# zju-vipa/ProtoPFormer

Measured on AMD Instinct MI355X. Metric: images/sec train step, deit_small+2000 protos, bs256, 1/2/4/8 MI355X, higher is better.
Workload: dtype bf16; 1 GPU; deit_small_patch16_224, synthetic 224x224, 2000x384 prototypes, 200 classes, k=81, batch 256/GPU (BASELINE.json configs[2]), train step = fwd+CE+PPC+bwd+allreduce+AdamW+EMA, DropPath 0.1; blocks after the token reservation run compacted on the 1+k reserved rows (equal to the masked full-length blocks to bf16 rounding); bf16 backbone: the reserved tokens differ from the fp32 reference's in ~2-3 % o; global_batch=256, parallelism=dp1

## Files before the change

include/ppf_hip.h:

```cpp
#ifndef PPF_HIP_H
#define PPF_HIP_H

#include <stddef.h>
#include <stdint.h>

#ifdef __cplusplus
extern "C" {
#endif

typedef struct ihipStream_t* ppf_stream_t;

#define PPF_ERR_SHAPE (-1)
#define PPF_ERR_ALIGN (-2)
#define PPF_ERR_ARG (-3)

#define PPF_ABI_VERSION 10

const char* ppf_last_error(void);
int ppf_abi_version(void);
int ppf_device_info(int* cu_count, int* clock_mhz, char* name, int name_len);
int ppf_stream_arm(ppf_stream_t stream, int on);
int ppf_stream_wait_stream(ppf_stream_t dst, ppf_stream_t src);
int64_t ppf_stream_mark(ppf_stream_t stream);
int ppf_stream_wait_mark(ppf_stream_t stream, int64_t ticket);

int ppf_gemm_bf16(const void* A, const void* B, void* C, int M, int N, int K, int lda, int ldb, int ldc, int trans_a,
                  int trans_b, int epi, const float* bias, const float* res, int ldres, const float* rowscale,
                  int rows_per_group, const float* colscale, const void* aux_in, void* aux_out, int ldaux, float* colsum,
                  float alpha, void* workspace, size_t workspace_bytes, ppf_stream_t stream);
size_t ppf_gemm_workspace_bytes(int M, int N, int K);

int ppf_gemm_test_force_g224(int force);

int ppf_gemm_probe(int enable);
int ppf_gemm_probe_read(double* ms_total, int64_t* launches, double* flops, double* bytes);

int ppf_path_probe(int enable);
int ppf_path_probe_read(int tag, double* ms_total, int64_t* launches, double* flops, double* bytes);

int ppf_gemm_bf16_batched(const void* A, const void* B, void* C, int M, int N, int K, int lda, int ldb, int ldc, int trans_a,
                          int trans_b, int out_f32, float alpha, int batch_outer, int batch_inner, int64_t sa_o, int64_t sa_i,
                          int64_t sb_o, int64_t sb_i, int64_t sc_o, int64_t sc_i, int kpad, ppf_stream_t stream);

int ppf_layernorm_bwd_f32(const float* dy, const float* x, const int* row_map, const float* w, const float* dres_in, float* dx_out, float* dw, float* db,
                          int rows, int D, float eps, ppf_stream_t stream);
int ppf_ew_bwd_f32(int kind, const float* a, const float* b, float* out, const float* rowscale, int rows_per_group, int M, int N, ppf_stream_t stream);
int ppf_colsum_f32(const float* in, float* out, int M, int N, ppf_stream_t stream);
int ppf_attn_bwd_f32(const float* qkv, const float* dout, const float* policy, float* dqkv, float* scratch, int B, int H, int N, int D, int self_keep,
                     int eps_n, ppf_stream_t stream);
int ppf_th_attn_bwd_f32(const float* qkv, const float* dout, const float* wl, const float* bl, const float* ww, const float* bw, float* dqkv,
                        float* dwl, float* dbl, float* dww, float* dbw, int B, int H, int N, int D, ppf_stream_t stream);
int ppf_class_attn_bwd_f32(const float* q, const float* k, const float* v, const float* policy, const float* dout, float* dq, float* dk, float* dv,
                           int B, int H, int N1, int D, ppf_stream_t stream);
// ... 163 lines not shown
```

protopformer_amd/_lib.py:

```python
import ctypes
import os

import torch

_HERE = os.path.dirname(os.path.abspath(__file__))
LIB_PATH = os.environ.get("PPF_LIB_PATH") or os.path.join(_HERE, "lib", "libppf_hip.so")

SIGS = {
    "ppf_gemm_bf16": "pppiiiiiiiiippipipppipf" "pz" "s",
    "ppf_device_info": "pppi",
    "ppf_rowgemm_bf16": "pp" "iiiiii" "pp" "s",
    "ppf_rowgemm_resid_ln": "pp" "iiiiii" "p" "pp" "pi" "pp" "pp" "ppp" "f" "s",
    "ppf_rowgemm_lnbwd": "pp" "iiiiii" "pppp" "ppp" "pi" "pp" "pz" "s",
    "ppf_rowgemm_colsum": "p" "iii" "ppp" "s",
    "ppf_layernorm_bwd_f32": "pppppppp" "ii" "f" "s",
    "ppf_ew_bwd_f32": "i" "ppp" "p" "i" "ii" "s",
    "ppf_colsum_f32": "pp" "ii" "s",
    "ppf_attn_bwd_f32": "ppppp" "iiiiii" "s",
    "ppf_th_attn_bwd_f32": "ppppppp" "pppp" "iiii" "s",
    "ppf_class_attn_bwd_f32": "pppppppp" "iiii" "s",
    "ppf_transpose_bf16_batched": "ppp" "ii" "s",
    "ppf_gemm_probe": "i",
    "ppf_gemm_test_force_g224": "i",
    "ppf_gemm_probe_read": "pppp",
    "ppf_path_probe": "i",
    "ppf_path_probe_read": "ipppp",
    "ppf_layernorm_fwd": "ppppppp" "iif" "s",
    "ppf_layernorm_bwd": "pppppp" "pppp" "pp" "i" "pppp" "ii" "pz" "s",
    "ppf_layernorm_bwd_reduce": "p" "ii" "pppp" "s",
    "ppf_cast_f32_bf16": "ppls",
    "ppf_cast_bf16_f32": "ppls",
    "ppf_im2col_patch": "ppiiiiis",
# ... 64 lines not shown

_CT = {"p": ctypes.c_void_p, "i": ctypes.c_int, "l": ctypes.c_int64, "L": ctypes.c_uint64, "f": ctypes.c_float, "s": ctypes.c_void_p, "z": ctypes.c_size_t}
_lib = None
_FAST = {}
_stream_override = []


def lib():
    global _lib
    if _lib is None:
        if not os.path.exists(LIB_PATH):
            raise RuntimeError(f"{LIB_PATH} not found: build it with `python -m protopformer_amd.build` "
                               "(there is no fallback path)")
        _lib = ctypes.CDLL(LIB_PATH)
        _lib.ppf_last_error.restype = ctypes.c_char_p
        _lib.ppf_abi_version.restype = ctypes.c_int
        got = _lib.ppf_abi_version()
        if got != EXPECTED_ABI:
            _lib = None
            raise RuntimeError(f"{LIB_PATH} was built for ABI version {got}, this binding expects {EXPECTED_ABI}: rebuild it with "
                               "`python -m protopformer_amd.build --force` (a stale library would receive shifted arguments)")
        _lib.ppf_gemm_workspace_bytes.restype = ctypes.c_size_t
        _lib.ppf_gemm_workspace_bytes.argtypes = [ctypes.c_int] * 3
        _lib.ppf_sgemm_pair_workspace.restype = ctypes.c_int64
        _lib.ppf_sgemm_pair_workspace.argtypes = [ctypes.c_int] * 5
        _lib.ppf_proto_bwd_single_workspace.restype = ctypes.c_size_t
        _lib.ppf_proto_bwd_single_workspace.argtypes = [ctypes.c_int] * 3
        _lib.ppf_proto_bwd_workspace.restype = ctypes.c_size_t
        _lib.ppf_proto_fwd_workspace.restype = ctypes.c_size_t
        _lib.ppf_proto_fwd_workspace.argtypes = [ctypes.c_int] * 2
        _lib.ppf_proto_bwd_workspace.argtypes = [ctypes.c_int] * 6
        _lib.ppf_layernorm_bwd_blocks.restype = ctypes.c_int
        _lib.ppf_layernorm_bwd_blocks.argtypes = [ctypes.c_int]
        _lib.ppf_sigmoid_bwd_blocks.restype = ctypes.c_int
        _lib.ppf_sigmoid_bwd_blocks.argtypes = [ctypes.c_int]
        _lib.ppf_clip_grad_blocks.restype = ctypes.c_int
        _lib.ppf_clip_grad_blocks.argtypes = []
        _lib.ppf_rowgemm_supported.restype = ctypes.c_int
        _lib.ppf_rowgemm_supported.argtypes = [ctypes.c_int] * 3
        _lib.ppf_attn_fwd_hm_supported.restype = ctypes.c_int
        _lib.ppf_attn_fwd_hm_supported.argtypes = [ctypes.c_int] * 3
        _lib.ppf_th_fused_supported.restype = ctypes.c_int
        _lib.ppf_th_fused_supported.argtypes = [ctypes.c_int] * 3
        _lib.ppf_th_grads_supported.restype = ctypes.c_int
        _lib.ppf_th_grads_supported.argtypes = [ctypes.c_int] * 3
        _lib.ppf_th_bwd_partial_floats.restype = ctypes.c_size_t
# ... 163 lines not shown
```

protopformer_amd/backbone.py:

```python
import functools
import os

import torch
import torch.nn as nn

from . import _lib, ops
from .ops import EPI_ATOMIC, EPI_BF16, EPI_DGELU, EPI_F32, EPI_GELU, EPI_RESID, EPI_SIGMOID_F32

LN_EPS = 1e-6
_KEEP_CACHE = {}
_ROW_BWD_MAX_ELEMS = 12_000_000


def _row_bwd(M, D):
    return M * D <= _ROW_BWD_MAX_ELEMS


def droppath_scales(rates, B, device, training):
    slots = [r if training else 0.0 for r in rates]
    active = [i for i, r in enumerate(slots) if r > 0.0]
    if not active:
        return None, [-1] * len(slots)
    key = (tuple(slots), str(device))
    st = _KEEP_CACHE.get(key)
# ... 153 lines not shown
        h = ops.linear_f32(h, c.weight, c.bias, kind=2 if j == len(convs) - 2 else 4)
    return h, acts


def addon_bwd(ppnet, store, head, f, df):
    convs = addon_convs(ppnet)
    gv = store.grad_view
    if len(convs) == 1:
        return ops.sigmoid_bwd(df, f, gv(convs[0].bias))
    acts = head["chain"]
    d = ops.ew_bwd_f32(1, df.contiguous(), f)
    for j in reversed(range(1, len(convs))):
        c, x_in = convs[j], acts[j - 1]
        ops.linear_wgrad_f32(d, x_in, gv(c.weight), gv(c.bias))
        d = ops.ew_bwd_f32(5, ops.linear_dgrad_f32(d, c.weight), x_in)
    ops.colsum_f32(d, gv(convs[0].bias))
    return ops.cast_bf16(d)


class WgradLane:

    def __init__(self, device):
        self.enabled = os.environ.get("PPF_WGRAD_STREAM", "1") != "0"
        self.streams = [torch.cuda.Stream(device=device)] if self.enabled else []
        self.raws = [st.cuda_stream for st in self.streams]
        self.last_read = {}
        self.tracked = set()
        self.held = []
        self.pending = []

    def track(self, t):
        self.tracked.add(t.data_ptr())
        return t

    def submit(self, fn, reads, tag=None, defer=False):
        if not self.enabled:
            fn()
            return
        self.pending.append((fn, reads, tag))
        self.held.extend(reads)
        if not defer:
            self.flush()

    def flush(self, tag=None):
        if not self.pending:
            return
        raw = self.raws[0]
        try:
            _lib.call("ppf_stream_wait_stream", raw, _lib.stream_ptr())
            for fn, reads, tg in self.pending:
                _lib.push_stream(raw)
                try:
                    fn()
                    ptrs = [t.data_ptr() for t in reads if t.data_ptr() in self.tracked]
                    if ptrs:
                        ticket = _lib.stream_mark(raw)
                        for q in ptrs:
                            self.last_read[q] = ticket
                finally:
                    _lib.pop_stream()
        finally:
            self.pending.clear()

    def before_overwrite(self, t):
        if t.data_ptr() not in self.tracked:
            raise RuntimeError("WgradLane.before_overwrite: buffer was not registered with track()")
        q = t.data_ptr()
        if any(r.data_ptr() == q for _, reads, _t in self.pending for r in reads):
            self.flush()
        ticket = self.last_read.pop(q, None)
        if ticket is not None:
            _lib.call("ppf_stream_wait_mark", _lib.stream_ptr(), ticket)

    def join(self):
        if self.enabled:
            self.flush()
            for raw in self.raws:
                _lib.call("ppf_stream_wait_stream", _lib.stream_ptr(), raw)
        self.last_read.clear()
        self.tracked.clear()
        self.held.clear()


def wgrad_lane(store):
    lane = getattr(store, "_wgrad_lane", None)
    if lane is None:
        lane = store._wgrad_lane = WgradLane(store.device)
    return lane


_ROLL_TAIL = 1
_ROLL_BATCH = 3


def _wgrad(store, dy16, x16, weight, bias=None, defer=False):
    gw = store.grad_view(weight)
    gb = store.grad_view(bias) if bias is not None else None
    wgrad_lane(store).submit(lambda: ops.gemm(dy16, x16, trans_a=True, trans_b=True, epi=EPI_ATOMIC, out=gw.reshape(weight.shape[0], -1),
                                              colsum=gb), (dy16, x16), defer=defer and min(weight.shape[0], weight.shape[1]) <= 256)


_DGRAD_ROW = 3


def _dgrad(store, dy16, weight, rows, which):
    wt = store.w16t(weight)
    if wt is not None and (_DGRAD_ROW & which) and ops.rowgemm_ok(wt.shape[0], wt.shape[1], rows):
        return ops.rowgemm_bf16(dy16, wt, rows)
    if wt is not None:
        return ops.gemm(dy16, wt, epi=EPI_BF16)
    return ops.gemm(dy16, store.w16(weight), trans_b=True, epi=EPI_BF16)


def head_bwd(ppnet, store, saved, df):
    head = saved["head"]
    conv = addon_convs(ppnet)[0]
    dz = addon_bwd(ppnet, store, head, saved["f"].reshape(-1, saved["f"].shape[-1]), df)
    _wgrad(store, dz, head["nf"], conv.weight)
    return ops.gemm(dz, store.w16(conv.weight).reshape(conv.out_channels, -1), trans_b=True, epi=EPI_BF16)


def chunk_ready(gs, lane, chunk):
# ... 187 lines not shown
```

protopformer_amd/csrc/gemm_bf16.hip:

```cpp
#include "ppf_common.h"
#include "gemm_common.h"
#include <cstdlib>
#include <utility>
#include <vector>

namespace {
using namespace ppfg;

constexpr int BM = 128, BN = 128, BK = 64, NTHREADS = 256;
constexpr int TILE_BYTES = BM * BK * 2;
constexpr int STAGE_LD = 68;
constexpr int STAGE_BYTES = 4 * 32 * STAGE_LD * 4;


__device__ __forceinline__ int lds_off_mode0(int r, int c16) { return r * 128 + ((c16 ^ ((r >> 1) & 7)) << 4); }
template <int ROWS>
__device__ __forceinline__ int lds_off_mode1(int kc, int col) {
    return kc * (ROWS * 2) + ((((col >> 5) ^ (kc & 3))) << 6) + ((col & 31) << 1);
}

typedef uint32_t u32x4 __attribute__((ext_vector_type(4)));

template <bool T, int ROWS>
struct TileIO {
// ... 94 lines not shown
            }
        }
    } else {
        const int col = (lane & 15) * 4;
        const int n = nbase + col;
        const EpiCols cc = epi_load_cols<EPI>(p, n, n < p.N);
        EpiRow rr[8];
#pragma unroll
        for (int pass = 0; pass < 8; ++pass) {
            const int m = mbase + pass * 4 + (lane >> 4);
            rr[pass] = epi_load_row<EPI>(p, m, n, m < p.M && n < p.N);
        }
#pragma unroll
        for (int pass = 0; pass < 8; ++pass) {
            const int r = pass * 4 + (lane >> 4);
            const int m = mbase + r;
            const float4 v = *reinterpret_cast<const float4*>(stage + r * STAGE_LD + col);
            if (m < p.M && n < p.N) epi_store<EPI>(p, m, n, v.x, v.y, v.z, v.w, cc, rr[pass]);
        }
    }
}

template <bool TA, bool TB, int EPI, bool COLSUM, int MT>
__global__ __launch_bounds__(NTHREADS, MT == 2 ? 3 : 2) void gemm_kernel(const GemmParams p_) {
    constexpr int PD = 1;
    extern __shared__ __attribute__((aligned(16))) unsigned char smem[];
    constexpr int TBM = 64 * MT;
    constexpr int A_BYTES = TBM * BK * 2;
    using IOA = TileIO<TA, TBM>;
    using IOB = TileIO<TB, BN>;
    const int tid = threadIdx.x, lane = tid & 63, wave = tid >> 6;
    const int wm = (wave & 1) * (32 * MT), wn = (wave >> 1) * 64;

    const int tiles_n = (p_.N + BN - 1) / BN;
    const int tiles = tiles_n * ((p_.M + TBM - 1) / TBM);
    const int vid_all = xcd_remap(blockIdx.x, gridDim.x);
    const int zslice = vid_all / tiles, vid = vid_all - zslice * tiles;
    const int m0 = (vid / tiles_n) * TBM, n0 = (vid % tiles_n) * BN;
    GemmParams p = p_;
    p.zslice = zslice;
    if (gridDim.y > 1) {
        const int bo = blockIdx.y / p.batch_inner, bi = blockIdx.y % p.batch_inner;
        p.A += bo * p.sa_o + bi * p.sa_i;
        p.B += bo * p.sb_o + bi * p.sb_i;
        const long long co = bo * p.sc_o + bi * p.sc_i;
        p.C = (EPI == EPI_BF16) ? (void*)(reinterpret_cast<bf16_t*>(p.C) + co) : (void*)(reinterpret_cast<float*>(p.C) + co);
    }

    const int nsplit = p.nsplit;
    const int kchunk = (((p.K + nsplit - 1) / nsplit) + BK - 1) / BK * BK;
    const int kbeg = zslice * kchunk;
    const int kend = min(p.K, kbeg + kchunk);
    if (kbeg >= kend) return;
    const int nk = (kend - kbeg + BK - 1) / BK;

    u32x4 ra[PD][IOA::NLD], rb[PD][IOB::NLD];
    unsigned ma[PD], mb[PD];
    f32x16 acc[2][MT];
#pragma unroll
// ... 70 lines not shown
#pragma unroll
    for (int mi = 0; mi < MT; ++mi) {
#pragma unroll
        for (int ni = 0; ni < 2; ++ni)
#pragma unroll
            for (int g = 0; g < 4; ++g)
                *reinterpret_cast<float4*>(stage + (lane & 31) * STAGE_LD + 32 * ni + 8 * g + 4 * h) =
                    make_float4(acc[ni][mi][4 * g], acc[ni][mi][4 * g + 1], acc[ni][mi][4 * g + 2], acc[ni][mi][4 * g + 3]);
        __builtin_amdgcn_wave_barrier();
        epilogue_rows<EPI>(p, stage, m0 + wm + 32 * mi, n0 + wn, lane);
        __builtin_amdgcn_wave_barrier();
        if constexpr (COLSUM) {
            const int m = m0 + wm + 32 * mi + (lane & 31);
            if (do_colsum && h == 0 && m < p.M) {
                if constexpr (EPI == EPI_PARTIAL) {
                    float* dst = p.ws + p.zslice * ((size_t)p.M * p.N + (size_t)p.cs_parts * p.M) + (size_t)p.M * p.N + m;
                    *dst = accs[mi][0];
                } else unsafeAtomicAdd(p.colsum + m, accs[mi][0]);
            }
        }
    }
}

template <int ROWS, int NTHR>
struct TileT {
    static constexpr int CPR = ROWS / 8;
    static constexpr int KPP = NTHR / CPR;
    static constexpr int NLD = BK / KPP;
    static __device__ __forceinline__ unsigned gload(u32x4 (&reg)[NLD], const bf16_t* __restrict__ X, int ld, int R, int row0, int k0, int kend, int tid) {
        const int c16 = tid % CPR, kb = tid / CPR;
        const int col = row0 + c16 * 8;
        const bool cok = (col + 8) <= R;
        const int cc = cok ? col : 0;
        unsigned mask = 0;
#pragma unroll
        for (int i = 0; i < NLD; ++i) {
            const int kc = k0 + kb + KPP * i;
            reg[i] = *reinterpret_cast<const u32x4*>(X + (size_t)min(kc, kend - 1) * ld + cc);
            mask |= (cok && kc < kend) ? (1u << i) : 0u;
        }
        return mask;
    }
    static __device__ __forceinline__ void sstore(const u32x4 (&reg)[NLD], unsigned mask, unsigned char* tile, int tid) {
        const u32x4 zero = {0u, 0u, 0u, 0u};
        const int c16 = tid % CPR, kb = tid / CPR;
#pragma unroll
        for (int i = 0; i < NLD; ++i)
            *reinterpret_cast<u32x4*>(tile + lds_off_mode1<ROWS>(kb + KPP * i, c16 * 8)) = ((mask >> i) & 1u) ? reg[i] : zero;
    }
    static __device__ __forceinline__ bf16x8 frag(const unsigned char* tile, int rbase, int ks, int lane) { return TileIO<true, ROWS>::frag(tile, rbase, ks, lane); }
};

template <int WMW, int WNW, bool COLSUM>
__global__ __launch_bounds__(64 * WMW * WNW, 1) void wgrad8_kernel(const GemmParams p_) {
    extern __shared__ __attribute__((aligned(16))) unsigned char smem[];
    constexpr int NTHR = 64 * WMW * WNW, TBM = 64 * WMW, TBN = 64 * WNW;
    using IOA = TileT<TBM, NTHR>;
    using IOB = TileT<TBN, NTHR>;
    const int tid = threadIdx.x, lane = tid & 63;
    const int wave = __builtin_amdgcn_readfirstlane(tid >> 6);
    const int wm = (wave % WMW) * 64, wn = (wave / WMW) * 64;
    const int tiles_n = (p_.N + TBN - 1) / TBN;
    const int tiles = tiles_n * ((p_.M + TBM - 1) / TBM);
    const int vid_all = xcd_remap(blockIdx.x, gridDim.x);
    const int zslice = vid_all / tiles, vid = vid_all - zslice * tiles;
    const int m0 = (vid / tiles_n) * TBM, n0 = (vid % tiles_n) * TBN;
    GemmParams p = p_;
    p.zslice = zslice;
    const int nsplit = p.nsplit;
    const int kchunk = (((p.K + nsplit - 1) / nsplit) + BK - 1) / BK * BK;
    const int kbeg = zslice * kchunk;
    const int kend = min(p.K, kbeg + kchunk);
    if (kbeg >= kend) return;
    const int nk = (kend - kbeg + BK - 1) / BK;

    u32x4 ra[IOA::NLD], rb[IOB::NLD];
    unsigned ma, mb;
    f32x16 acc[2][2];
#pragma unroll
    for (int i = 0; i < 2; ++i)
#pragma unroll
        for (int j = 0; j < 2; ++j)
#pragma unroll
            for (int r = 0; r < 16; ++r) acc[i][j][r] = 0.f;
    f32x16 accs[2];
    if constexpr (COLSUM) {
#pragma unroll
// ... 44 lines not shown
        __syncthreads();
    }
    const int h = lane >> 5;
    float* stage = reinterpret_cast<float*>(smem) + wave * (32 * STAGE_LD);
#pragma unroll
    for (int mi = 0; mi < 2; ++mi) {
#pragma unroll
        for (int ni = 0; ni < 2; ++ni)
#pragma unroll
            for (int g = 0; g < 4; ++g)
                *reinterpret_cast<float4*>(stage + (lane & 31) * STAGE_LD + 32 * ni + 8 * g + 4 * h) =
                    make_float4(acc[ni][mi][4 * g], acc[ni][mi][4 * g + 1], acc[ni][mi][4 * g + 2], acc[ni][mi][4 * g + 3]);
        __builtin_amdgcn_wave_barrier();
        epilogue_rows<EPI_PARTIAL>(p, stage, m0 + wm + 32 * mi, n0 + wn, lane);
        __builtin_amdgcn_wave_barrier();
        if constexpr (COLSUM) {
            const int m = m0 + wm + 32 * mi + (lane & 31);
            if (do_colsum && h == 0 && m < p.M) {
                float* dst = p.ws + p.zslice * ((size_t)p.M * p.N + (size_t)p.cs_parts * p.M) + (size_t)p.M * p.N + m;
                *dst = accs[mi][0];
            }
        }
    }
}

template <int WMW, int WNW>
int launch_wgrad8(const GemmParams& p, int splitk, hipStream_t stream) {
    auto kern = wgrad8_kernel<WMW, WNW, true>;
    constexpr int NTHR = 64 * WMW * WNW, TBM = 64 * WMW, TBN = 64 * WNW;
    constexpr int opnd = (TBM + TBN) * BK * 2, strips = (NTHR / 64) * 32 * STAGE_LD * 4;
    constexpr int lds = opnd > strips ? opnd : strips;
    static bool attr_set = false;
    if (!attr_set) {
        hipError_t e = hipFuncSetAttribute(reinterpret_cast<const void*>(kern), hipFuncAttributeMaxDynamicSharedMemorySize, lds);
        if (e != hipSuccess) { ppf_set_error("hipFuncSetAttribute(wgrad8): %s", hipGetErrorString(e)); return (int)e; }
        attr_set = true;
    }
    const int tiles = ((p.M + TBM - 1) / TBM) * ((p.N + TBN - 1) / TBN);
    hipLaunchKernelGGL(kern, dim3(tiles * splitk), dim3(NTHR), lds, stream, p);
    PPF_LAUNCH_CHECK();
    return 0;
}

typedef __attribute__((address_space(3))) void g4_lds_t;
typedef const __attribute__((address_space(1))) void g4_gbl_t;

// ... 212 lines not shown
    constexpr int TBM = 64 * MT;
    const int tiles = ((p.M + TBM - 1) / TBM) * ((p.N + BN - 1) / BN);
    auto kern = gemm_kernel<TA, TB, EPI, COLSUM, MT>;
    constexpr int opnd = TBM * BK * 2 + TILE_BYTES;
    constexpr int lds = opnd > STAGE_BYTES ? opnd : STAGE_BYTES;
    static bool attr_set = false;
    if (!attr_set) {
        hipError_t e = hipFuncSetAttribute(reinterpret_cast<const void*>(kern), hipFuncAttributeMaxDynamicSharedMemorySize, lds);
        if (e != hipSuccess) { ppf_set_error("hipFuncSetAttribute(gemm): %s", hipGetErrorString(e)); return (int)e; }
        attr_set = true;
    }
    GemmParams q = p;
    q.nsplit = splitk;
    hipLaunchKernelGGL(kern, dim3(tiles * splitk, nbatch, 1), dim3(NTHREADS), lds, stream, q);
    PPF_LAUNCH_CHECK();
    return 0;
}

template <bool TA, bool TB, int EPI, bool COLSUM>
int launch(const GemmParams& p, int splitk, hipStream_t stream, int nbatch = 1) {
    return launch_impl<TA, TB, EPI, COLSUM, 2>(p, splitk, stream, nbatch);
}

__global__ __launch_bounds__(256) void splitk_reduce_kernel(const float* __restrict__ ws, float* __restrict__ C, float* __restrict__ colsum,
                                                            int M, int N, int ldc, int nsplit, int cs_parts) {
    const size_t mn = (size_t)M * N, slice = mn + (colsum ? (size_t)cs_parts * M : 0);
    const size_t total4 = mn / 4;
    const size_t i = (size_t)blockIdx.x * 256 + threadIdx.x;
    if (i < total4) {
        const float* p = ws + i * 4;
        float4 acc = make_float4(0.f, 0.f, 0.f, 0.f);
        for (int z0 = 0; z0 < nsplit; z0 += 16) {
            float4 v[16];
#pragma unroll
            for (int u = 0; u < 16; ++u) {
                const int z = min(z0 + u, nsplit - 1);
                v[u] = *reinterpret_cast<const float4*>(p + (size_t)z * slice);
            }
#pragma unroll
            for (int u = 0; u < 16; ++u)
                if (z0 + u < nsplit) { acc.x += v[u].x; acc.y += v[u].y; acc.z += v[u].z; acc.w += v[u].w; }
        }
        const size_t e = i * 4, m = e / N, n = e - m * N;
        float4* dst = reinterpret_cast<float4*>(C + m * ldc + n);
        const float4 c = *dst;
        *dst = make_float4(c.x + acc.x, c.y + acc.y, c.z + acc.z, c.w + acc.w);
    } else if (colsum && i < total4 + (size_t)M) {
        const size_t m = i - total4;
        float a = 0.f;
        for (int z = 0; z < nsplit; ++z)
            for (int q = 0; q < cs_parts; ++q) a += ws[(size_t)z * slice + mn + (size_t)q * M + m];
        colsum[m] += a;
    }
}

struct Probe {
    bool on = false;
    std::vector<std::pair<hipEvent_t, hipEvent_t>> pool;
    size_t used = 0;
    double flops = 0.0, bytes = 0.0;
    std::pair<hipEvent_t, hipEvent_t> acquire() {
        if (used == pool.size()) {
            hipEvent_t a = nullptr, b = nullptr;
            const unsigned fl = hipEventDisableSystemFence;
            (void)hipEventCreateWithFlags(&a, fl); (void)hipEventCreateWithFlags(&b, fl);
            pool.emplace_back(a, b);
        }
        return pool[used++];
    }
};
Probe g_probe;

constexpr size_t PPF_GEMM_COUNTER_BYTES = 16384;

int pick_splitk(int M, int N, int K) {
    const int tiles = ((M + BM - 1) / BM) * ((N + BN - 1) / BN);
    const int target = min(M, N) <= 256 ? 216 : 432;
    int s = target / tiles;
    const int maxs = (K + 4 * BK - 1) / (4 * BK);
    if (s > maxs) s = maxs;
    if (s < 1) s = 1;
    const int kchunk = (((K + s - 1) / s) + BK - 1) / BK * BK;
    return (K + kchunk - 1) / kchunk;
}

}

extern "C" {

int ppf_gemm_test_force_g224(int force) { g_force_g224 = force != 0; return 0; }

size_t ppf_gemm_workspace_bytes(int M, int N, int K) {
    return PPF_GEMM_COUNTER_BYTES + (size_t)pick_splitk(M, N, K) * ((size_t)M * N + M) * sizeof(float);
}

int ppf_gemm_bf16(const void* A, const void* B, void* C, int M, int N, int K, int lda, int ldb, int ldc, int trans_a,
                  int trans_b, int epi, const float* bias, const float* res, int ldres, const float* rowscale,
                  int rows_per_group, const float* colscale, const void* aux_in, void* aux_out, int ldaux, float* colsum,
                  float alpha, void* workspace, size_t workspace_bytes, hipStream_t stream) {
    PPF_CHECK_ARG(M > 0 && N > 0 && K > 0, PPF_ERR_SHAPE, "ppf_gemm_bf16: bad shape M=%d N=%d K=%d", M, N, K);
    PPF_CHECK_ARG((lda % 8) == 0 && (ldb % 8) == 0 && (ldc % 4) == 0 && (N % 4) == 0, PPF_ERR_ALIGN,
                  "ppf_gemm_bf16: lda/ldb must be multiples of 8, ldc and N of 4 (lda=%d ldb=%d ldc=%d N=%d)", lda, ldb, ldc, N);
    PPF_CHECK_ARG(trans_a ? (M % 8 == 0) : (K % 8 == 0), PPF_ERR_ALIGN, "ppf_gemm_bf16: A inner extent must be a multiple of 8");
    PPF_CHECK_ARG(trans_b ? (N % 8 == 0) : (K % 8 == 0), PPF_ERR_ALIGN, "ppf_gemm_bf16: B inner extent must be a multiple of 8");
    PPF_CHECK_ARG((((uintptr_t)A | (uintptr_t)B | (uintptr_t)C) & 15) == 0, PPF_ERR_ALIGN, "ppf_gemm_bf16: pointers must be 16-byte aligned");
    PPF_CHECK_ARG(!(trans_a && !trans_b), PPF_ERR_ARG, "ppf_gemm_bf16: (trans_a=1, trans_b=0) is not instantiated");
    PPF_CHECK_ARG((((uintptr_t)aux_in | (uintptr_t)aux_out | (uintptr_t)res) & 15) == 0 && (ldaux % 4) == 0 && (ldres % 4) == 0, PPF_ERR_ALIGN,
// ... 24 lines not shown
            case EPI_SIGMOID_F32: return launch<false, false, EPI_SIGMOID_F32, false>(p, 1, stream);
            case EPI_RESID: return launch<false, false, EPI_RESID, false>(p, 1, stream);
            case EPI_DGELU: return launch<false, false, EPI_DGELU, false>(p, 1, stream);
            default: break;
        }
    } else if (!trans_a && trans_b) {
        switch (epi) {
            case EPI_BF16: return launch<false, true, EPI_BF16, false>(p, 1, stream);
            case EPI_F32: return launch<false, true, EPI_F32, false>(p, 1, stream);
            case EPI_DGELU: return launch<false, true, EPI_DGELU, false>(p, 1, stream);
            default: break;
        }
    } else {
        switch (epi) {
            case EPI_ATOMIC: {
                const int ns = pick_splitk(M, N, K);
                const size_t need = PPF_GEMM_COUNTER_BYTES + (size_t)ns * ((size_t)M * N + M) * sizeof(float);
                if (workspace == nullptr || workspace_bytes < need || ns == 1) return launch<true, true, EPI_ATOMIC, true>(p, ns, stream);
                p.ws = (float*)((unsigned char*)workspace + PPF_GEMM_COUNTER_BYTES);
                p.cs_parts = 1;
                p.nsplit = ns;
                hipEvent_t e0 = nullptr, e1 = nullptr;
                if (g_probe.on) { auto ev = g_probe.acquire(); e0 = ev.first; e1 = ev.second; (void)hipEventRecord(e0, stream); }
                const bool wide = (M < N ? M : N) >= 320;
                int rc;
                if (wide && M >= 512 && M >= N && (M % 256 == 0 || M >= 1024)) rc = launch_wgrad8<4, 2>(p, ns, stream);
                else if (wide && N >= 512 && (N % 256 == 0 || N >= 1024)) rc = launch_wgrad8<2, 4>(p, ns, stream);
                else rc = launch<true, true, EPI_PARTIAL, true>(p, ns, stream);
                if (rc) return rc;
                if (g_probe.on) {
                    (void)hipEventRecord(e1, stream);
                    g_probe.flops += 2.0 * M * N * (double)K;
                    g_probe.bytes += 2.0 * ((double)M * K + (double)N * K) + 4.0 * M * N;
                }
                const size_t work = (size_t)M * N / 4 + (colsum ? M : 0);
                const int grid = (int)((work + 255) / 256);
                hipLaunchKernelGGL(splitk_reduce_kernel, dim3(grid), dim3(256), 0, stream, p.ws, (float*)C, colsum, M, N, ldc, ns, p.cs_parts);
                PPF_LAUNCH_CHECK();
                return 0;
            }
            case EPI_F32: return launch<true, true, EPI_F32, false>(p, 1, stream);
            default: break;
        }
    }
    ppf_set_error("ppf_gemm_bf16: combination trans_a=%d trans_b=%d epi=%d not instantiated", trans_a, trans_b, epi);
    return PPF_ERR_ARG;
}

int ppf_gemm_probe(int enable) {
    if (enable == 1) { g_probe.used = 0; g_probe.flops = 0.0; g_probe.bytes = 0.0; }
    if (enable == 2) {
        for (auto& e : g_probe.pool) { (void)hipEventDestroy(e.first); (void)hipEventDestroy(e.second); }
        g_probe.pool.clear(); g_probe.used = 0;
    }
    g_probe.on = enable == 1;
    return 0;
}
int ppf_gemm_probe_read(double* ms_total, int64_t* launches, double* flops, double* bytes) {
    double ms = 0.0;
    for (size_t i = 0; i < g_probe.used; ++i) {
        auto& e = g_probe.pool[i];
        float t = 0.f;
        hipError_t rc = hipEventSynchronize(e.second);
        if (rc == hipSuccess) rc = hipEventElapsedTime(&t, e.first, e.second);
        if (rc != hipSuccess) { ppf_set_error("ppf_gemm_probe_read: %s", hipGetErrorString(rc)); return (int)rc; }
        ms += t;
    }
    if (ms_total) *ms_total = ms;
    if (launches) *launches = (int64_t)g_probe.used;
// ... 39 lines not shown
```

protopformer_amd/ops.py:

```python
import os

import torch

from . import _lib

EPI_BF16, EPI_F32, EPI_GELU, EPI_SIGMOID_F32, EPI_RESID, EPI_DGELU, EPI_ATOMIC = range(7)


DOMINANT_NAME = ("weight-gradient bf16 MFMA GEMM, split over the contraction, ordered partial tiles: wgrad8_kernel<4,2> / <2,4> (256x128 / 128x256 tiles) "
                 "and gemm_kernel<TA=1,TB=1,EPI_PARTIAL,COLSUM> (128x128)")


_WORKSPACE = {}


def _workspace(device, nbytes):
    key = (device, _lib.stream_ptr())
    buf = _WORKSPACE.get(key)
    if buf is None or buf.numel() < nbytes:
        if buf is not None:
            _RETIRED_WS.append(buf)
        buf = torch.empty(max(nbytes, 64 << 20), dtype=torch.uint8, device=device)
        _WORKSPACE[key] = buf
    return buf


_GEMM_WS = {}
_RETIRED_WS = []


def _gemm_workspace(device, nbytes):
    key = (device, _lib.stream_ptr())
    buf = _GEMM_WS.get(key)
# ... 17 lines not shown
    _chk(a, torch.bfloat16), _chk(b, torch.bfloat16)
    lda = a.shape[1] if lda is None else lda
    ldb = b.shape[1] if ldb is None else ldb
    M, K = (a.shape[1], a.numel() // lda) if trans_a else (a.numel() // lda, a.shape[1])
    N, Kb = (b.shape[1], b.numel() // ldb) if trans_b else (b.numel() // ldb, b.shape[1])
    assert K == Kb, f"contraction mismatch {K} vs {Kb}"
    if out is None:
        odt = torch.float32 if epi in (EPI_F32, EPI_SIGMOID_F32, EPI_RESID, EPI_ATOMIC) else torch.bfloat16
        out = torch.empty((M, N), dtype=odt, device=a.device)
        if epi == EPI_ATOMIC:
            zero_(out)
    ldaux = 0
    for t in (aux_in, aux_out):
        if t is not None:
            _chk(t, torch.uint8 if epi in (EPI_GELU, EPI_DGELU) else torch.bfloat16)
            ldaux = t.shape[-1]
    ws = None
    if epi == EPI_ATOMIC and workspace:
        ws = _gemm_workspace(a.device, _lib.lib().ppf_gemm_workspace_bytes(M, N, K))
    _lib.call("ppf_gemm_bf16", a, b, out, M, N, K, lda, ldb, out.shape[-1], int(trans_a), int(trans_b), epi,
              bias, res, res.shape[-1] if res is not None else 0, rowscale, rows_per_group, colscale, aux_in, aux_out, ldaux,
              colsum, float(alpha), ws, ws.numel() if ws is not None else 0)
    return out


def rowgemm_ok(D, K, rows_per_tile):
    return bool(_lib.lib().ppf_rowgemm_supported(int(D), int(K), int(rows_per_tile)))


_CU_COUNT = {}


def rowgemm_tile_rows(M, rows_per_sample, device=None, backward=False):
    dev = torch.cuda.current_device() if device is None else device
    cus = _CU_COUNT.get(dev)
    if cus is None:
        cus = _CU_COUNT[dev] = torch.cuda.get_device_properties(dev).multi_processor_count
    tiles = (M + rows_per_sample - 1) // rows_per_sample
    if 3 * tiles > 2 * cus or rows_per_sample <= 16:
        return rows_per_sample
    half = (rows_per_sample + 1) // 2
    if backward:
        target = max(1, int(0.62 * cus))
        return max(half, min(rows_per_sample, (M + target - 1) // target))
    return half

# ... 666 lines not shown
```

Before: 17530 images/sec.

## Fuse pairs of weight-gradient GEMMs into one grouped split-K launch

Adds a paired weight-gradient kernel that runs two split-K GEMMs in a single grid, splitting the blocks between them, followed by one combined split-K reduction kernel. The split factors are chosen jointly, in proportion to each problem's FLOPs, against a CU-sized slot target. The wgrad lane now defers submissions and merges adjacent jobs into pairs. This cuts launch count and lets small GEMMs share the device instead of each underfilling it. In exchange, jobs are held back longer on the side stream, which may reduce overlap, and the new split factors and larger workspace may be less tuned than the single-GEMM heuristics.

```diff
diff --git a/include/ppf_hip.h b/include/ppf_hip.h
--- a/include/ppf_hip.h
+++ b/include/ppf_hip.h
@@ -29,6 +29,12 @@
                   int rows_per_group, const float* colscale, const void* aux_in, void* aux_out, int ldaux, float* colsum,
                   float alpha, void* workspace, size_t workspace_bytes, ppf_stream_t stream);
 size_t ppf_gemm_workspace_bytes(int M, int N, int K);
+
+int ppf_gemm_bf16_wgrad_pair(const void* A0, const void* B0, void* C0, int M0, int N0, int K0, int lda0, int ldb0, int ldc0, float* colsum0,
+                             const void* A1, const void* B1, void* C1, int M1, int N1, int K1, int lda1, int ldb1, int ldc1, float* colsum1,
+                             void* workspace, size_t workspace_bytes, ppf_stream_t stream);
+size_t ppf_gemm_workspace_pair_bytes(int M0, int N0, int K0, int M1, int N1, int K1);
+int ppf_gemm_test_pair_target(int target);
 
 int ppf_gemm_test_force_g224(int force);
 
diff --git a/protopformer_amd/_lib.py b/protopformer_amd/_lib.py
--- a/protopformer_amd/_lib.py
+++ b/protopformer_amd/_lib.py
@@ -8,6 +8,8 @@
 
 SIGS = {
     "ppf_gemm_bf16": "pppiiiiiiiiippipipppipf" "pz" "s",
+    "ppf_gemm_bf16_wgrad_pair": "ppp" "iiiiii" "p" "ppp" "iiiiii" "p" "pz" "s",
+    "ppf_gemm_test_pair_target": "i",
     "ppf_device_info": "pppi",
     "ppf_rowgemm_bf16": "pp" "iiiiii" "pp" "s",
     "ppf_rowgemm_resid_ln": "pp" "iiiiii" "p" "pp" "pi" "pp" "pp" "ppp" "f" "s",
@@ -118,6 +120,8 @@
                                "`python -m protopformer_amd.build --force` (a stale library would receive shifted arguments)")
         _lib.ppf_gemm_workspace_bytes.restype = ctypes.c_size_t
         _lib.ppf_gemm_workspace_bytes.argtypes = [ctypes.c_int] * 3
+        _lib.ppf_gemm_workspace_pair_bytes.restype = ctypes.c_size_t
+        _lib.ppf_gemm_workspace_pair_bytes.argtypes = [ctypes.c_int] * 6
         _lib.ppf_sgemm_pair_workspace.restype = ctypes.c_int64
         _lib.ppf_sgemm_pair_workspace.argtypes = [ctypes.c_int] * 5
         _lib.ppf_proto_bwd_single_workspace.restype = ctypes.c_size_t
diff --git a/protopformer_amd/backbone.py b/protopformer_amd/backbone.py
--- a/protopformer_amd/backbone.py
+++ b/protopformer_amd/backbone.py
@@ -199,6 +199,7 @@
 
     def __init__(self, device):
         self.enabled = os.environ.get("PPF_WGRAD_STREAM", "1") != "0"
+        self.pair = self.enabled and os.environ.get("PPF_WGRAD_PAIR", "1") != "0"
         self.streams = [torch.cuda.Stream(device=device)] if self.enabled else []
         self.raws = [st.cuda_stream for st in self.streams]
         self.last_read = {}
@@ -210,11 +211,20 @@
         self.tracked.add(t.data_ptr())
         return t
 
-    def submit(self, fn, reads, tag=None, defer=False):
+    def submit(self, fn, reads, tag=None, defer=False, job=None):
         if not self.enabled:
             fn()
             return
-        self.pending.append((fn, reads, tag))
+        if job is not None and self.pair:
+            i = next((j for j in reversed(range(len(self.pending))) if self.pending[j][3] is not None), None)
+            if i is not None:
+                _, reads0, _, job0 = self.pending.pop(i)
+                fn, reads, job = (lambda a=job0, b=job: ops.wgrad_pair(*a, *b)), tuple(reads0) + tuple(r for r in reads if all(r is not q for q in reads0)), None
+            elif not defer:
+                job = None
+        else:
+            job = None
+        self.pending.append((fn, reads, tag, job))
         self.held.extend(reads)
         if not defer:
             self.flush()
@@ -225,7 +235,7 @@
         raw = self.raws[0]
         try:
             _lib.call("ppf_stream_wait_stream", raw, _lib.stream_ptr())
-            for fn, reads, tg in self.pending:
+            for fn, reads, tg, _job in self.pending:
                 _lib.push_stream(raw)
                 try:
                     fn()
@@ -243,7 +253,7 @@
         if t.data_ptr() not in self.tracked:
             raise RuntimeError("WgradLane.before_overwrite: buffer was not registered with track()")
         q = t.data_ptr()
-        if any(r.data_ptr() == q for _, reads, _t in self.pending for r in reads):
+        if any(r.data_ptr() == q for _, reads, _t, _job in self.pending for r in reads):
             self.flush()
         ticket = self.last_read.pop(q, None)
         if ticket is not None:
@@ -273,8 +283,10 @@
 def _wgrad(store, dy16, x16, weight, bias=None, defer=False):
     gw = store.grad_view(weight)
     gb = store.grad_view(bias) if bias is not None else None
-    wgrad_lane(store).submit(lambda: ops.gemm(dy16, x16, trans_a=True, trans_b=True, epi=EPI_ATOMIC, out=gw.reshape(weight.shape[0], -1),
-                                              colsum=gb), (dy16, x16), defer=defer and min(weight.shape[0], weight.shape[1]) <= 256)
+    lane = wgrad_lane(store)
+    out = gw.reshape(weight.shape[0], -1)
+    lane.submit(lambda: ops.gemm(dy16, x16, trans_a=True, trans_b=True, epi=EPI_ATOMIC, out=out, colsum=gb), (dy16, x16),
+                defer=defer and (lane.pair or min(weight.shape[0], weight.shape[1]) <= 256), job=(dy16, x16, out, gb))
 
 
 _DGRAD_ROW = 3
diff --git a/protopformer_amd/csrc/gemm_bf16.hip b/protopformer_amd/csrc/gemm_bf16.hip
--- a/protopformer_amd/csrc/gemm_bf16.hip
+++ b/protopformer_amd/csrc/gemm_bf16.hip
@@ -140,7 +140,7 @@
 }
 
 template <bool TA, bool TB, int EPI, bool COLSUM, int MT>
-__global__ __launch_bounds__(NTHREADS, MT == 2 ? 3 : 2) void gemm_kernel(const GemmParams p_) {
+__device__ __forceinline__ void gemm_body(const GemmParams& p_, const int bid, const int nbid) {
     constexpr int PD = 1;
     extern __shared__ __attribute__((aligned(16))) unsigned char smem[];
     constexpr int TBM = 64 * MT;
@@ -152,7 +152,7 @@
 
     const int tiles_n = (p_.N + BN - 1) / BN;
     const int tiles = tiles_n * ((p_.M + TBM - 1) / TBM);
-    const int vid_all = xcd_remap(blockIdx.x, gridDim.x);
+    const int vid_all = xcd_remap(bid, nbid);
     const int zslice = vid_all / tiles, vid = vid_all - zslice * tiles;
     const int m0 = (vid / tiles_n) * TBM, n0 = (vid % tiles_n) * BN;
     GemmParams p = p_;
@@ -269,6 +269,11 @@
     }
 }
 
+template <bool TA, bool TB, int EPI, bool COLSUM, int MT>
+__global__ __launch_bounds__(NTHREADS, MT == 2 ? 3 : 2) void gemm_kernel(const GemmParams p_) {
+    gemm_body<TA, TB, EPI, COLSUM, MT>(p_, blockIdx.x, gridDim.x);
+}
+
 template <int ROWS, int NTHR>
 struct TileT {
     static constexpr int CPR = ROWS / 8;
@@ -299,7 +304,7 @@
 };
 
 template <int WMW, int WNW, bool COLSUM>
-__global__ __launch_bounds__(64 * WMW * WNW, 1) void wgrad8_kernel(const GemmParams p_) {
+__device__ __forceinline__ void wgrad8_body(const GemmParams& p_, const int bid, const int nbid) {
     extern __shared__ __attribute__((aligned(16))) unsigned char smem[];
     constexpr int NTHR = 64 * WMW * WNW, TBM = 64 * WMW, TBN = 64 * WNW;
     using IOA = TileT<TBM, NTHR>;
@@ -309,7 +314,7 @@
     const int wm = (wave % WMW) * 64, wn = (wave / WMW) * 64;
     const int tiles_n = (p_.N + TBN - 1) / TBN;
     const int tiles = tiles_n * ((p_.M + TBM - 1) / TBM);
-    const int vid_all = xcd_remap(blockIdx.x, gridDim.x);
+    const int vid_all = xcd_remap(bid, nbid);
     const int zslice = vid_all / tiles, vid = vid_all - zslice * tiles;
     const int m0 = (vid / tiles_n) * TBM, n0 = (vid % tiles_n) * TBN;
     GemmParams p = p_;
@@ -400,6 +405,11 @@
             }
         }
     }
+}
+
+template <int WMW, int WNW, bool COLSUM>
+__global__ __launch_bounds__(64 * WMW * WNW, 1) void wgrad8_kernel(const GemmParams p_) {
+    wgrad8_body<WMW, WNW, COLSUM>(p_, blockIdx.x, gridDim.x);
 }
 
 template <int WMW, int WNW>
@@ -658,11 +668,50 @@
     return launch_impl<TA, TB, EPI, COLSUM, 2>(p, splitk, stream, nbatch);
 }
 
-__global__ __launch_bounds__(256) void splitk_reduce_kernel(const float* __restrict__ ws, float* __restrict__ C, float* __restrict__ colsum,
-                                                            int M, int N, int ldc, int nsplit, int cs_parts) {
+struct PairParams { GemmParams p0, p1; int wg0; };
+
+template <int KIND>
+__device__ __forceinline__ void wgrad_tile_body(const GemmParams& p, const int bid, const int nbid) {
+    if constexpr (KIND == 0) gemm_body<true, true, EPI_PARTIAL, true, 2>(p, bid, nbid);
+    else if constexpr (KIND == 1) wgrad8_body<4, 2, true>(p, bid, nbid);
+    else wgrad8_body<2, 4, true>(p, bid, nbid);
+}
+
+template <int KIND0, int KIND1>
+__global__ __launch_bounds__(KIND0 == 0 ? 256 : 512, KIND0 == 0 ? 3 : 1) void wgrad_pair_kernel(const PairParams pp) {
+    static_assert((KIND0 == 0) == (KIND1 == 0), "both problems of a pair run with the same workgroup size");
+    const int bid = blockIdx.x;
+    if (bid < pp.wg0) wgrad_tile_body<KIND0>(pp.p0, bid, pp.wg0);
+    else wgrad_tile_body<KIND1>(pp.p1, bid - pp.wg0, (int)gridDim.x - pp.wg0);
+}
+
+inline int pair_tiles(int kind, int M, int N) {
+    const int tm = kind == 1 ? 256 : 128, tn = kind == 2 ? 256 : 128;
+    return ((M + tm - 1) / tm) * ((N + tn - 1) / tn);
+}
+
+template <int KIND0, int KIND1>
+int launch_wgrad_pair(const PairParams& pp, int wg1, hipStream_t stream) {
+    auto kern = wgrad_pair_kernel<KIND0, KIND1>;
+    constexpr int nthr = KIND0 == 0 ? 256 : 512;
+    constexpr int opnd = KIND0 == 0 ? 2 * TILE_BYTES : 3 * TILE_BYTES, strips = (nthr / 64) * 32 * STAGE_LD * 4;
+    constexpr int lds = opnd > strips ? opnd : strips;
+    static bool attr_set = false;
+    if (!attr_set) {
+        hipError_t e = hipFuncSetAttribute(reinterpret_cast<const void*>(kern), hipFuncAttributeMaxDynamicSharedMemorySize, lds);
+        if (e != hipSuccess) { ppf_set_error("hipFuncSetAttribute(wgrad_pair): %s", hipGetErrorString(e)); return (int)e; }
+        attr_set = true;
+    }
+    hipLaunchKernelGGL(kern, dim3(pp.wg0 + wg1), dim3(nthr), lds, stream, pp);
+    PPF_LAUNCH_CHECK();
+    return 0;
+}
+
+__device__ __forceinline__ void splitk_reduce_body(const float* __restrict__ ws, float* __restrict__ C, float* __restrict__ colsum,
+                                                   int M, int N, int ldc, int nsplit, int cs_parts, const int bid) {
     const size_t mn = (size_t)M * N, slice = mn + (colsum ? (size_t)cs_parts * M : 0);
     const size_t total4 = mn / 4;
-    const size_t i = (size_t)blockIdx.x * 256 + threadIdx.x;
+    const size_t i = (size_t)bid * 256 + threadIdx.x;
     if (i < total4) {
         const float* p = ws + i * 4;
         float4 acc = make_float4(0.f, 0.f, 0.f, 0.f);
@@ -688,6 +737,18 @@
             for (int q = 0; q < cs_parts; ++q) a += ws[(size_t)z * slice + mn + (size_t)q * M + m];
         colsum[m] += a;
     }
+}
+
+__global__ __launch_bounds__(256) void splitk_reduce_kernel(const float* __restrict__ ws, float* __restrict__ C, float* __restrict__ colsum,
+                                                            int M, int N, int ldc, int nsplit, int cs_parts) {
+    splitk_reduce_body(ws, C, colsum, M, N, ldc, nsplit, cs_parts, blockIdx.x);
+}
+
+struct ReduceArgs { const float* ws; float* C; float* colsum; int M, N, ldc, nsplit; };
+__global__ __launch_bounds__(256) void splitk_reduce_pair_kernel(const ReduceArgs a, const ReduceArgs b, const int g0) {
+    const int bid = blockIdx.x;
+    if (bid < g0) splitk_reduce_body(a.ws, a.C, a.colsum, a.M, a.N, a.ldc, a.nsplit, 1, bid);
+    else splitk_reduce_body(b.ws, b.C, b.colsum, b.M, b.N, b.ldc, b.nsplit, 1, bid - g0);
 }
 
 struct Probe {
@@ -719,6 +780,36 @@
     const int kchunk = (((K + s - 1) / s) + BK - 1) / BK * BK;
     return (K + kchunk - 1) / kchunk;
 }
+
+int g_pair_target = 0;
+void pick_splitk_pair(const int (&M)[2], const int (&N)[2], const int (&K)[2], int (&s)[2]) {
+    const int narrow = min(min(M[0], N[0]), min(M[1], N[1])) <= 256;
+    const int target = g_pair_target > 0 ? g_pair_target : (narrow ? 216 : 432);
+    const double f0 = (double)M[0] * N[0] * K[0], f1 = (double)M[1] * N[1] * K[1];
+    const double slots[2] = {target * f0 / (f0 + f1), target * f1 / (f0 + f1)};
+    for (int i = 0; i < 2; ++i) {
+        const int tiles = ((M[i] + BM - 1) / BM) * ((N[i] + BN - 1) / BN);
+        int si = (int)(slots[i] / tiles + 0.5);
+        const int maxs = (K[i] + 4 * BK - 1) / (4 * BK);
+        if (si > maxs) si = maxs;
+        if (si < 1) si = 1;
+        const int kchunk = (((K[i] + si - 1) / si) + BK - 1) / BK * BK;
+        s[i] = (K[i] + kchunk - 1) / kchunk;
+    }
+}
+
+int wgrad_kind(int M, int N) {
+    const bool wide = (M < N ? M : N) >= 320;
+    if (wide && M >= 512 && M >= N && (M % 256 == 0 || M >= 1024)) return 1;
+    if (wide && N >= 512 && (N % 256 == 0 || N >= 1024)) return 2;
+    return 0;
+}
+void pair_kinds(const int (&M)[2], const int (&N)[2], int (&kind)[2]) {
+    kind[0] = wgrad_kind(M[0], N[0]); kind[1] = wgrad_kind(M[1], N[1]);
+    if (kind[0] == 0 || kind[1] == 0) kind[0] = kind[1] = 0;
+}
+
+size_t pair_slab_floats(int M, int N, int s) { return (size_t)s * ((size_t)M * N + M); }
 
 }
 
@@ -789,10 +880,10 @@
                 p.nsplit = ns;
                 hipEvent_t e0 = nullptr, e1 = nullptr;
                 if (g_probe.on) { auto ev = g_probe.acquire(); e0 = ev.first; e1 = ev.second; (void)hipEventRecord(e0, stream); }
-                const bool wide = (M < N ? M : N) >= 320;
+                const int kind = wgrad_kind(M, N);
                 int rc;
-                if (wide && M >= 512 && M >= N && (M % 256 == 0 || M >= 1024)) rc = launch_wgrad8<4, 2>(p, ns, stream);
-                else if (wide && N >= 512 && (N % 256 == 0 || N >= 1024)) rc = launch_wgrad8<2, 4>(p, ns, stream);
+                if (kind == 1) rc = launch_wgrad8<4, 2>(p, ns, stream);
+                else if (kind == 2) rc = launch_wgrad8<2, 4>(p, ns, stream);
                 else rc = launch<true, true, EPI_PARTIAL, true>(p, ns, stream);
                 if (rc) return rc;
                 if (g_probe.on) {
@@ -812,6 +903,89 @@
     }
     ppf_set_error("ppf_gemm_bf16: combination trans_a=%d trans_b=%d epi=%d not instantiated", trans_a, trans_b, epi);
     return PPF_ERR_ARG;
+}
+
+int ppf_gemm_test_pair_target(int target) { g_pair_target = target > 0 ? target : 0; return 0; }
+
+size_t ppf_gemm_workspace_pair_bytes(int M0, int N0, int K0, int M1, int N1, int K1) {
+    if (M0 <= 0 || N0 <= 0 || K0 <= 0 || M1 <= 0 || N1 <= 0 || K1 <= 0) return 0;
+    const int M[2] = {M0, M1}, N[2] = {N0, N1}, K[2] = {K0, K1};
+    int s[2];
+    pick_splitk_pair(M, N, K, s);
+    return PPF_GEMM_COUNTER_BYTES + (pair_slab_floats(M0, N0, s[0]) + pair_slab_floats(M1, N1, s[1])) * sizeof(float);
+}
+
+int ppf_gemm_bf16_wgrad_pair(const void* A0, const void* B0, void* C0, int M0, int N0, int K0, int lda0, int ldb0, int ldc0, float* colsum0,
+                             const void* A1, const void* B1, void* C1, int M1, int N1, int K1, int lda1, int ldb1, int ldc1, float* colsum1,
+                             void* workspace, size_t workspace_bytes, hipStream_t stream) {
+    const void* A[2] = {A0, A1}; const void* B[2] = {B0, B1}; void* C[2] = {C0, C1};
+    const int M[2] = {M0, M1}, N[2] = {N0, N1}, K[2] = {K0, K1}, lda[2] = {lda0, lda1}, ldb[2] = {ldb0, ldb1}, ldc[2] = {ldc0, ldc1};
+    float* colsum[2] = {colsum0, colsum1};
+    for (int i = 0; i < 2; ++i) {
+        PPF_CHECK_ARG(M[i] > 0 && N[i] > 0 && K[i] > 0, PPF_ERR_SHAPE, "ppf_gemm_bf16_wgrad_pair: bad shape M=%d N=%d K=%d", M[i], N[i], K[i]);
+        PPF_CHECK_ARG((lda[i] % 8) == 0 && (ldb[i] % 8) == 0 && (ldc[i] % 4) == 0 && (M[i] % 8) == 0 && (N[i] % 8) == 0, PPF_ERR_ALIGN,
+                      "ppf_gemm_bf16_wgrad_pair: lda/ldb/M/N must be multiples of 8, ldc of 4 (lda=%d ldb=%d ldc=%d M=%d N=%d)", lda[i], ldb[i], ldc[i], M[i], N[i]);
+        PPF_CHECK_ARG(lda[i] >= M[i] && ldb[i] >= N[i] && ldc[i] >= N[i], PPF_ERR_ARG, "ppf_gemm_bf16_wgrad_pair: a leading dimension is shorter than its row");
+        PPF_CHECK_ARG((((uintptr_t)A[i] | (uintptr_t)B[i] | (uintptr_t)C[i]) & 15) == 0 && A[i] && B[i] && C[i], PPF_ERR_ALIGN,
+                      "ppf_gemm_bf16_wgrad_pair: pointers must be non-null and 16-byte aligned");
+    }
+    int s[2];
+    pick_splitk_pair(M, N, K, s);
+    const size_t fl0 = pair_slab_floats(M[0], N[0], s[0]), fl1 = pair_slab_floats(M[1], N[1], s[1]);
+    const size_t need = PPF_GEMM_COUNTER_BYTES + (fl0 + fl1) * sizeof(float);
+    if (workspace == nullptr || workspace_bytes < need || (((uintptr_t)workspace) & 15) != 0) {
+        for (int i = 0; i < 2; ++i) {
+            const int rc = ppf_gemm_bf16(A[i], B[i], C[i], M[i], N[i], K[i], lda[i], ldb[i], ldc[i], 1, 1, EPI_ATOMIC, nullptr, nullptr, 0, nullptr, 1, nullptr,
+                                         nullptr, nullptr, 0, colsum[i], 1.0f, workspace, workspace_bytes, stream);
+            if (rc) return rc;
+        }
+        return 0;
+    }
+    int kind[2];
+    pair_kinds(M, N, kind);
+    float* ws0 = (float*)((unsigned char*)workspace + PPF_GEMM_COUNTER_BYTES);
+    float* wsp[2] = {ws0, ws0 + fl0};
+    PairParams pp;
+    GemmParams* gp[2] = {&pp.p0, &pp.p1};
+    for (int i = 0; i < 2; ++i) {
+        GemmParams& p = *gp[i];
+        p.A = (const bf16_t*)A[i]; p.B = (const bf16_t*)B[i]; p.C = C[i]; p.M = M[i]; p.N = N[i]; p.K = K[i]; p.lda = lda[i]; p.ldb = ldb[i]; p.ldc = ldc[i];
+        p.bias = nullptr; p.res = nullptr; p.ldres = 0; p.rowscale = nullptr; p.rows_per_group = 1; p.colscale = nullptr; p.aux_in = nullptr;
+        p.aux_out = nullptr; p.ldaux = 0; p.colsum = colsum[i]; p.alpha = 1.0f; p.ws = wsp[i];
+        p.batch_inner = 1; p.sa_o = p.sa_i = p.sb_o = p.sb_i = p.sc_o = p.sc_i = 0; p.kpad = 0; p.cs_parts = 1; p.nsplit = s[i]; p.zslice = 0;
+    }
+    pp.wg0 = pair_tiles(kind[0], M[0], N[0]) * s[0];
+    const int wg1 = pair_tiles(kind[1], M[1], N[1]) * s[1];
+    hipEvent_t e0 = nullptr, e1 = nullptr;
+    if (g_probe.on) { auto ev = g_probe.acquire(); e0 = ev.first; e1 = ev.second; (void)hipEventRecord(e0, stream); }
+    int rc;
+    const int key = kind[0] * 4 + kind[1];
+    switch (key) {
+        case 0: rc = launch_wgrad_pair<0, 0>(pp, wg1, stream); break;
+        case 5: rc = launch_wgrad_pair<1, 1>(pp, wg1, stream); break;
+        case 6: rc = launch_wgrad_pair<1, 2>(pp, wg1, stream); break;
+        case 9: rc = launch_wgrad_pair<2, 1>(pp, wg1, stream); break;
+        case 10: rc = launch_wgrad_pair<2, 2>(pp, wg1, stream); break;
+        default: ppf_set_error("ppf_gemm_bf16_wgrad_pair: tile forms %d + %d not instantiated", kind[0], kind[1]); return PPF_ERR_ARG;
+    }
+    if (rc) return rc;
+    if (g_probe.on) {
+        (void)hipEventRecord(e1, stream);
+        for (int i = 0; i < 2; ++i) {
+            g_probe.flops += 2.0 * M[i] * N[i] * (double)K[i];
+            g_probe.bytes += 2.0 * ((double)M[i] * K[i] + (double)N[i] * K[i]) + 4.0 * M[i] * N[i];
+        }
+    }
+    ReduceArgs ra[2];
+    int grid[2];
+    for (int i = 0; i < 2; ++i) {
+        ra[i] = ReduceArgs{wsp[i], (float*)C[i], colsum[i], M[i], N[i], ldc[i], s[i]};
+        const size_t work = (size_t)M[i] * N[i] / 4 + (colsum[i] ? M[i] : 0);
+        grid[i] = (int)((work + 255) / 256);
+    }
+    hipLaunchKernelGGL(splitk_reduce_pair_kernel, dim3(grid[0] + grid[1]), dim3(256), 0, stream, ra[0], ra[1], grid[0]);
+    PPF_LAUNCH_CHECK();
+    return 0;
 }
 
 int ppf_gemm_probe(int enable) {
diff --git a/protopformer_amd/ops.py b/protopformer_amd/ops.py
--- a/protopformer_amd/ops.py
+++ b/protopformer_amd/ops.py
@@ -8,7 +8,7 @@
 
 
 DOMINANT_NAME = ("weight-gradient bf16 MFMA GEMM, split over the contraction, ordered partial tiles: wgrad8_kernel<4,2> / <2,4> (256x128 / 128x256 tiles) "
-                 "and gemm_kernel<TA=1,TB=1,EPI_PARTIAL,COLSUM> (128x128)")
+                 "and gemm_kernel<TA=1,TB=1,EPI_PARTIAL,COLSUM> (128x128); two of them in one grid where they are issued in pairs (wgrad_pair_kernel)")
 
 
 _WORKSPACE = {}
@@ -72,6 +72,18 @@
               bias, res, res.shape[-1] if res is not None else 0, rowscale, rows_per_group, colscale, aux_in, aux_out, ldaux,
               colsum, float(alpha), ws, ws.numel() if ws is not None else 0)
     return out
+
+
+def wgrad_pair(dy0, x0, out0, colsum0, dy1, x1, out1, colsum1, workspace=None):
+    dims = []
+    for dy, x, out in ((dy0, x0, out0), (dy1, x1, out1)):
+        _chk(dy, torch.bfloat16), _chk(x, torch.bfloat16), _chk(out, torch.float32)
+        assert dy.shape[0] == x.shape[0] and tuple(out.shape) == (dy.shape[1], x.shape[1]), "wgrad_pair: out must be [dy columns, x columns]"
+        dims.append((dy.shape[1], x.shape[1], dy.shape[0]))
+    (M0, N0, K0), (M1, N1, K1) = dims
+    ws = workspace if workspace is not None else _gemm_workspace(dy0.device, _lib.lib().ppf_gemm_workspace_pair_bytes(M0, N0, K0, M1, N1, K1))
+    _lib.call("ppf_gemm_bf16_wgrad_pair", dy0, x0, out0, M0, N0, K0, M0, N0, N0, colsum0, dy1, x1, out1, M1, N1, K1, M1, N1, N1, colsum1,
+              ws, ws.numel())
 
 
 def rowgemm_ok(D, K, rows_per_tile):
```

After: 17600 images/sec (median of 3 runs). No clear change (+0.4%).
